# UCSD-Comp-Imaging/Nerf-Simple

Measured on AMD Instinct MI355X. Metric: ray-samples/sec at 800x800x128, higher is better.
Workload: dtype f16

## Files before the change

### nerf-simple_amd/csrc/mlp_bf16_16.hip

```cpp
#include "composite_device.h"
#include "launchers.h"

using namespace nerf_layout;

#ifdef NERF_HALF
typedef _Float16 elem_t;
#define NERF_MFMA __builtin_amdgcn_mfma_f32_16x16x32_f16
#define NERF_KERNEL nerf_mlp_f16_16_kernel
#define NERF_LAUNCH nerf_amd_launch_mlp_f16_16
#else
typedef __bf16 elem_t;
#define NERF_MFMA __builtin_amdgcn_mfma_f32_16x16x32_bf16
#define NERF_KERNEL nerf_mlp_bf16_16_kernel
#define NERF_LAUNCH nerf_amd_launch_mlp_bf16_16
#endif
#include "mlp16_chain.h"

namespace {

#ifdef NERF_HALF
constexpr bool FOLD = true;
#else
constexpr bool FOLD = false;
#endif
struct MlpPlan {
    static constexpr int LAYERS = NUM_LAYERS;
    static constexpr bool SAVE = !FOLD;
    static constexpr int tpc(int L) { return L == 0 ? 8 : 4; }
    static constexpr int mt(int L) { return FOLD ? fold_mt(L) : b16_mt(L); }
    static constexpr int layer_off_kib(int L) { return FOLD ? fold_layer_off_kib(L) : b16_layer_off_kib(L); }
    static constexpr int bias_off(int L) { return FOLD ? fold_bias_off(L) : b16_bias_off(L); }
};
static_assert(NUM_CHUNKS<MlpPlan> == (FOLD ? 34 : 38) && plan_fits<MlpPlan>(), "chunks per tile / weight buffer, parity");

constexpr int LDS_POSD = LDS_CHAIN_END;
constexpr int LDS_POSX = LDS_POSD + WAVES * NCB * 1024;
constexpr int LDS_TOTAL = LDS_POSX + WAVES * NCB * 2048;
constexpr int RING_PTS = 1024;
constexpr int LDS_RING_RAW = LDS_TOTAL;
constexpr int LDS_RING_T = LDS_RING_RAW + RING_PTS * 16;
constexpr int LDS_TOTAL_COMP = LDS_RING_T + RING_PTS * 4;
constexpr int COMP_MAX_N = RING_PTS - TILE_PTS;
static_assert(COMP_MAX_N == FUSED_RENDER_MAX_N, "api.hip routes by this limit");
static_assert(LDS_TOTAL_COMP <= 160 * 1024, "LDS budget");
static_assert((RING_PTS & (RING_PTS - 1)) == 0 && RING_PTS % TILE_PTS == 0, "ring indexing");

static_assert(ACT_TILE_PTS == TILE_PTS && MASK_TILE_PTS == TILE_PTS, "activation blocks and mask tiles are the kernel's tiles");

struct State {
    using Plan = MlpPlan;
    ex8 X[NCB][8], Y[NCB][8];
    f32x4 pend[NCB][2];
    float sigma[NCB], rgb[NCB][3];
    bool bad;
    unsigned posd_off[NCB];
    char* acts;
    long long P;
    long long tile;
    int loff[NCB];
    unsigned mb[NCB][2];
    float amax[4];
    long long mask_tile;
    long long p_end;
    unsigned ring_q0;
    WFrag* wf;
};

template <bool RAYS, int SAVE, bool COMP>
__device__ __forceinline__ void stage_inputs(const Ctx& c, const MlpArgs& a, long long tile_base, State& st) {
    const int col = c.lane & 15, g = c.lane >> 4;
    float u_mine = 0.f;
    bool dev_rng = false;
    long long b0 = 0;
    int r0 = 0;
    if constexpr (RAYS) {
        b0 = tile_base / a.N;
        r0 = (int)(tile_base - b0 * a.N);
    }
    const long long p_end = COMP ? st.p_end : a.P;
    const int last_local = (int)(p_end - 1 - tile_base);
    constexpr bool RAY_POSD = RAYS && !SAVE;
    if constexpr (RAY_POSD) {
        const int top = last_local < TILE_PTS - 1 ? last_local : TILE_PTS - 1;
        const int nrays = (int)(split_point(b0, r0, top, a.N).b - b0) + 1;
        for (int idx = threadIdx.x; idx < nrays * 32; idx += WAVES * 64) {
            const int ray = idx >> 5, slot = idx & 31, gg = slot >> 3, sl = slot & 7;
            const float* rp = a.rays + (b0 + ray) * 6 + 3;
            const float dx = rp[0], dy = rp[1], dz = rp[2];
            const float nrm = norm3(dx, dy, dz);
            float val = 0.f;
            if (sl < 6) {
                const int cd = sl >> 1;
                const float dc = __fdiv_rn(cd == 0 ? dx : cd == 1 ? dy : dz, nrm);
                val = enc_lane(to_revolutions(dc), 2 * gg + (sl & 1));
            } else if (sl == 6 && gg < 3) {
                val = __fdiv_rn(gg == 0 ? dx : gg == 1 ? dy : dz, nrm);
            }
            lds_store<elem_t>(LDS_POSD + ray * 64 + slot * 2, 0, (elem_t)val);
        }
    }
    if constexpr (RAYS && NCB == 2) {
        dev_rng = (a.flags & NERF_FLAG_DEVICE_RNG) && !(a.flags & NERF_FLAG_TS_GIVEN);
        if (dev_rng) {
            int lm = c.wave * 32 + (c.lane & 31);
            if (lm > last_local) lm = last_local;
            u_mine = device_rng_uniform(a, split_point(b0, r0, lm, a.N));
        }
    }
#pragma unroll
    for (int cb = 0; cb < NCB; ++cb) {
        long long p = tile_base + c.wave * (16 * NCB) + cb * 16 + col;
        const bool valid = p < p_end;
        st.loff[cb] = valid ? block_lane_offset(g, c.wave * (16 * NCB) + cb * 16 + col) : LOFF_INVALID;
        if constexpr (SAVE == 2) {
            if (cb == 0)
                st.loff[0] = tile_base + c.wave * 32 + 16 * (c.lane >> 5) + col < p_end ? f8_lane_offset(c.lane, c.wave) : LOFF_INVALID;
        }
        if (!valid) p = p_end - 1;
        PointIn pt;
        st.posd_off[cb] = c.b_posd + cb * 1024;
        if constexpr (RAYS) {
            const float u_cb = (NCB == 2) ? __shfl(u_mine, cb * 16 + col) : 0.f;
            int lp = c.wave * (16 * NCB) + cb * 16 + col;
            if (lp > last_local) lp = last_local;
            if (SAVE && a.pts) {
                pt = fetch_point_pts(a, p);
            } else {
                const RaySample rs = split_point(b0, r0, lp, a.N);
                if constexpr (RAY_POSD) st.posd_off[cb] = LDS_POSD + (unsigned)(rs.b - b0) * 64 + g * 16;
                pt = fetch_point_rays<!RAY_POSD>(a, p, rs, u_cb, dev_rng);
                if constexpr (COMP) {
                    if (valid && g == 0)
                        lds_store<float>(((st.ring_q0 + c.wave * (16 * NCB) + cb * 16 + col) & (RING_PTS - 1)) * 4, LDS_RING_T, pt.t);
                }
                if (valid && g == 0 && a.ts_out) a.ts_out[p] = pt.t;
            }
        } else {
            pt = fetch_point_pts(a, p);
        }
        {
            const float xyz[3] = {pt.x, pt.y, pt.z};
            float v[16];
#pragma unroll
            for (int cd = 0; cd < 3; ++cd) {
                const TwoF q = to_revolutions(xyz[cd]);
#pragma unroll
                for (int jj = 0; jj < 5; ++jj) v[cd * 5 + jj] = enc_lane(q, 5 * g + jj);
            }
            v[15] = g == 0 ? pt.x : g == 1 ? pt.y : g == 2 ? pt.z : 0.f;
#pragma unroll
            for (int e = 0; e < 2; ++e) {
                u32x4 r;
#pragma unroll
                for (int i = 0; i < 4; ++i) r[i] = pack2<false>(v[8 * e + 2 * i], v[8 * e + 2 * i + 1]);
                lds_store<u32x4>(c.b_posx, cb * 2048 + e * 1024, r);
            }
        }
        if constexpr (!RAY_POSD) {
            const float dd[3] = {pt.d1, pt.d2, pt.d3};
            float v[8];
#pragma unroll
            for (int cd = 0; cd < 3; ++cd) {
                const TwoF q = to_revolutions(dd[cd]);
#pragma unroll
                for (int jj = 0; jj < 2; ++jj) v[cd * 2 + jj] = enc_lane(q, 2 * g + jj);
            }
            v[6] = g == 0 ? pt.d1 : g == 1 ? pt.d2 : g == 2 ? pt.d3 : 0.f;
            v[7] = 0.f;
            u32x4 r;
#pragma unroll
            for (int i = 0; i < 4; ++i) r[i] = pack2<false>(v[2 * i], v[2 * i + 1]);
            lds_store<u32x4>(c.b_posd, cb * 1024, r);
        }
    }
}

template <bool RAYS, int SAVE, bool COMP>
__device__ __forceinline__ void run_tile(const Ctx& c, const MlpArgs& a, long long tile_base, State& st) {
    stage_inputs<RAYS, SAVE, COMP>(c, a, tile_base, st);
    run_layer<0, SAVE>(c, st, st.X, st.X);
    run_layer<1, SAVE>(c, st, st.X, st.Y);
    run_layer<2, SAVE>(c, st, st.Y, st.X);
    run_layer<3, SAVE>(c, st, st.X, st.Y);
    run_layer<4, SAVE>(c, st, st.Y, st.X);
    run_layer<5, SAVE>(c, st, st.X, st.Y);
    run_layer<6, SAVE>(c, st, st.Y, st.X);
    run_layer<7, SAVE>(c, st, st.X, st.Y);
    ex8 (&c_in)[NCB][8] = FOLD ? st.Y : st.X;
    ex8 (&c_out)[NCB][8] = FOLD ? st.X : st.Y;
    run_layer<8, SAVE>(c, st, st.Y, st.X);
    run_layer<9, SAVE>(c, st, c_in, c_out);
    run_layer<10, SAVE>(c, st, c_out, c_in);
    epilogue_piece<10, 0>(0, st.pend, st.X, st);
    for (int cb_ = 1; cb_ < NCB; ++cb_) epilogue_piece<10, 0>(4 * cb_, st.pend, st.X, st);
}

__device__ __forceinline__ bool finite4(float x, float y, float z, float w) {
    return __builtin_fabsf(x) + __builtin_fabsf(y) + __builtin_fabsf(z) + __builtin_fabsf(w) < __builtin_inff();
}

struct RingSamples {
    unsigned q0;
    __device__ __forceinline__ float t(int i) const {
        return lds_load<float>(((q0 + (unsigned)i) & (RING_PTS - 1)) * 4, LDS_RING_T);
    }
    __device__ __forceinline__ f32x4 c(int i) const {
        return lds_load<f32x4>(((q0 + (unsigned)i) & (RING_PTS - 1)) * 16, LDS_RING_RAW);
    }
};

template <bool RAYS, int SAVE, bool COMP>
__device__ __forceinline__ void kernel_body(const MlpArgs& a, long long ntiles) {
    static_assert(!COMP || (RAYS && !SAVE), "the fused render is the rays-mode inference kernel");
    using P = MlpPlan;
    Ctx c;
    c.wave = __builtin_amdgcn_readfirstlane(threadIdx.x >> 6);
    c.lane = threadIdx.x & 63;
    const char* img = reinterpret_cast<const char*>(a.packed);
    c.wrsrc = __builtin_amdgcn_make_buffer_rsrc(const_cast<char*>(img), 0, (int)B16_IMAGE_BYTES, 0x00020000);
    c.wave_goff = c.wave * 1024;
    c.lane16 = c.lane * 16;
#pragma unroll
    for (int p = 0; p < 2; ++p) {
        c.b_wread[p] = LDS_W0 + p * LDS_WBUF + c.lane * 16;
        c.s_wdst[p] = LDS_W0 + p * LDS_WBUF + c.wave * 1024;
    }
    c.b_bias = (c.lane >> 4) * 16;
    c.b_posx = LDS_POSX + c.wave * (NCB * 2048) + c.lane * 16;
    c.b_posd = LDS_POSD + c.wave * (NCB * 1024) + c.lane * 16;

    {
        const float* bsrc = reinterpret_cast<const float*>(img + (long long)B16_WEIGHT_KIB * 1024);
        for (int i = threadIdx.x; i < B16_BIAS_FLOATS; i += WAVES * 64)
            lds_store<float>(i * 4, LDS_BIAS, bsrc[i]);
        Stage<P, NUM_CHUNKS<P> - 1>::issue(c);
    }
    asm volatile("s_waitcnt vmcnt(0)" ::: "memory");
    __syncthreads();
    WFrag wf;
    {
        constexpr int F0 = chunk_tiles<P>(0) * (layer_desc(0).chain_k / 32 + layer_desc(0).extra_slots / 32);
#pragma unroll
        for (int f = 0; f < 4 && f < F0; ++f) wf.a[f] = lds_load<ex8>(c.b_wread[0], f * 1024);
        wf.bias0 = lds_load<f32x4>(c.b_bias, LDS_BIAS + P::bias_off(0) * 4);
    }

    if constexpr (!COMP) {
        for (long long tile = blockIdx.x; tile < ntiles; tile += gridDim.x) {
            const long long tile_base = tile * TILE_PTS;
            asm volatile("" : "+s"(c.wave_goff));
            State st;
            st.wf = &wf;
            st.acts = reinterpret_cast<char*>(a.acts);
            st.P = a.P;
            st.mask_tile = SAVE == 2 ? f8_mask_offset_bytes(0, tile, 0, a.P) : mask_offset_bytes(0, tile, 0, a.P);
            st.tile = tile;
            st.bad = false;
            run_tile<RAYS, SAVE, false>(c, a, tile_base, st);
            bool bad = st.bad;
            if (c.lane < 16) {
#pragma unroll
                for (int cb = 0; cb < NCB; ++cb) {
                    const long long p = tile_base + c.wave * (16 * NCB) + cb * 16 + c.lane;
                    if (p < a.P) {
                        const f32x4 o = {st.rgb[cb][0], st.rgb[cb][1], st.rgb[cb][2], st.sigma[cb]};
                        *reinterpret_cast<f32x4*>(a.raw + p * 4) = o;
                        bad |= !finite4(o[0], o[1], o[2], o[3]);
                    }
                }
            }
            flag_nonfinite(c, bad);
        }
    } else {
        const long long B = a.P / a.N;
        const long long r_lo = (long long)blockIdx.x * B / gridDim.x, r_hi = ((long long)blockIdx.x + 1) * B / gridDim.x;
        const long long range_base = r_lo * a.N;
        const int n_pts = (int)((r_hi - r_lo) * a.N);
        const nerf_composite::RayOut out{a.rgb, a.disp, a.alpha, a.acc, a.w, a.pixels};
        int next_ray = 0, n_complete = 0;
        for (int q_tile = 0; q_tile < n_pts; q_tile += TILE_PTS) {
            const long long tile_base = range_base + q_tile;
            asm volatile("" : "+s"(c.wave_goff));
            State st;
            st.wf = &wf;
            st.acts = nullptr;
            st.P = a.P;
            st.mask_tile = 0;
            st.tile = 0;
            st.p_end = range_base + n_pts;
            st.ring_q0 = (unsigned)q_tile & (RING_PTS - 1);
            st.bad = false;
            run_tile<true, false, true>(c, a, tile_base, st);
            bool bad = st.bad;
            if (c.lane < 16) {
#pragma unroll
                for (int cb = 0; cb < NCB; ++cb) {
                    const int local = c.wave * (16 * NCB) + cb * 16 + c.lane;
                    if (q_tile + local < n_pts) {
                        const f32x4 o = {st.rgb[cb][0], st.rgb[cb][1], st.rgb[cb][2], st.sigma[cb]};
                        lds_store<f32x4>(((st.ring_q0 + local) & (RING_PTS - 1)) * 16, LDS_RING_RAW, o);
                        bad |= !finite4(o[0], o[1], o[2], o[3]);
                    }
                }
            }
            flag_nonfinite(c, bad);
            asm volatile("s_waitcnt lgkmcnt(0)" ::: "memory");
            __builtin_amdgcn_s_barrier();
            asm volatile("" ::: "memory");
            const int done_q = q_tile + TILE_PTS < n_pts ? q_tile + TILE_PTS : n_pts;
            while ((n_complete + 1) * a.N <= done_q) ++n_complete;
            if (n_complete - next_ray >= WAVES || done_q + TILE_PTS - next_ray * a.N > RING_PTS || done_q == n_pts) {
                for (int ray = next_ray + c.wave; ray < n_complete; ray += WAVES) {
                    const long long gray = r_lo + ray;
                    const float* d = a.rays + gray * 6 + 3;
                    const float dnorm = nerf_composite::unit_dir_norm(d[0], d[1], d[2], true);
                    const RingSamples src{(unsigned)(ray * a.N) & (RING_PTS - 1)};
                    nerf_composite::composite_ray(src, a.N, c.lane, dnorm, gray, out);
                }
                next_ray = n_complete;
                asm volatile("s_waitcnt lgkmcnt(0)" ::: "memory");
                __builtin_amdgcn_s_barrier();
                asm volatile("" ::: "memory");
            }
        }
    }
}

template <bool RAYS, bool SAVE, bool COMP>
__global__ __launch_bounds__(WAVES * 64, WAVES / 4) void NERF_KERNEL(MlpArgs a, long long ntiles) {
    extern __shared__ __attribute__((aligned(16))) char smem[];
    (void)smem;
    kernel_body<RAYS, SAVE ? 1 : 0, COMP>(a, ntiles);
}
#ifndef NERF_HALF
__global__ __launch_bounds__(WAVES * 64, WAVES / 4) void nerf_mlp_train_e4m3_kernel(MlpArgs a, long long ntiles) {
    extern __shared__ __attribute__((aligned(16))) char smem[];
    (void)smem;
    kernel_body<true, 2, false>(a, ntiles);
}
#endif

}

extern "C" int NERF_LAUNCH(const MlpArgs* args, int rays_mode, hipStream_t stream) {
    (void)hipGetLastError();
    MlpArgs a = *args;
    if (a.P <= 0) return 0;
    const long long ntiles = (a.P + TILE_PTS - 1) / TILE_PTS;
    const int cus = device_cus();
    const long long grid = ntiles < cus ? ntiles : cus;
    hipError_t e = hipSuccess;
    const bool comp = a.rgb || a.disp || a.acc || a.alpha || a.w || a.pixels;
    if (comp) {
        if (!rays_mode || a.acts || a.N > COMP_MAX_N || a.P / grid + a.N >= (1ll << 31)) return -2;
        auto kern = NERF_KERNEL<true, false, true>;
        e = allow_dynamic_lds(reinterpret_cast<const void*>(kern), LDS_TOTAL_COMP);
        if (e != hipSuccess) return (int)e;
        hipLaunchKernelGGL(kern, dim3((unsigned)grid), dim3(WAVES * 64), LDS_TOTAL_COMP, stream, a, ntiles);
        return (int)hipGetLastError();
    }
#ifdef NERF_HALF
    if (a.acts) return -2;
    auto kern = rays_mode ? NERF_KERNEL<true, false, false> : NERF_KERNEL<false, false, false>;
#else
    if (a.acts && !rays_mode) return -2;
    if ((a.flags & NERF_FLAG_STORE_E4M3) && !a.acts) return -2;
    auto kern = a.acts ? ((a.flags & NERF_FLAG_STORE_E4M3) ? nerf_mlp_train_e4m3_kernel : NERF_KERNEL<true, true, false>)
                       : (rays_mode ? NERF_KERNEL<true, false, false> : NERF_KERNEL<false, false, false>);
#endif
    e = allow_dynamic_lds(reinterpret_cast<const void*>(kern), LDS_TOTAL);
    if (e != hipSuccess) return (int)e;
    hipLaunchKernelGGL(kern, dim3((unsigned)grid), dim3(WAVES * 64), LDS_TOTAL, stream, a, ntiles);
    return (int)hipGetLastError();
}
```

### nerf-simple_amd/csrc/nerf_device.h

```cpp
#pragma once
#include <hip/hip_runtime.h>
#include <stdint.h>
#include <atomic>
#include "nerf_layout.h"

typedef __bf16 bf16x8 __attribute__((ext_vector_type(8)));
typedef __bf16 bf16x2 __attribute__((ext_vector_type(2)));
typedef short s16x2 __attribute__((ext_vector_type(2)));
typedef unsigned short u16x2 __attribute__((ext_vector_type(2)));
typedef float f32x2 __attribute__((ext_vector_type(2)));
typedef float f32x4 __attribute__((ext_vector_type(4)));
typedef float f32x16 __attribute__((ext_vector_type(16)));
typedef unsigned u32x4 __attribute__((ext_vector_type(4)));

#define NERF_FLAG_TS_GIVEN 1u
#define NERF_FLAG_DEVICE_RNG 2u
#define NERF_FLAG_SEED_IN_MEMORY 4u
#define NERF_FLAG_STORE_E4M3 8u

struct MlpArgs {
    const float* pts;
    const float* rays;
    const float* u;
    const float* tbins;
    const void* packed;
    float* raw;
    float* ts_out;
    void* acts;
    long long P;
    long long ray_id0;
    unsigned long long seed;
    int N;
    unsigned flags;
    float* rgb;
    float* disp;
    float* alpha;
    float* acc;
    float* w;
    float* pixels;
};

struct DensityArgs {
    const float* pts;
    long long stride;
    const void* packed;
    float* sigma;
    long long P;
    long long ny, nz;
    float lo[3], step[3];
};

constexpr int NERF_MAX_DEVICES = 64;
inline int device_cus() {
    static int cache[NERF_MAX_DEVICES] = {};
    int dev = 0;
    if (hipGetDevice(&dev) != hipSuccess || dev < 0 || dev >= NERF_MAX_DEVICES) return 256;
    if (cache[dev] == 0) {
        int cus = 256;
        if (hipDeviceGetAttribute(&cus, hipDeviceAttributeMultiprocessorCount, dev) != hipSuccess || cus <= 0) cus = 256;
        cache[dev] = cus;
    }
    return cache[dev];
}
inline hipError_t allow_dynamic_lds(const void* kernel, int bytes) {
    struct Slot { const void* kernel; int dev; };
    static Slot slots[128];
    static std::atomic<int> used{0};
    int dev = 0;
    if (hipGetDevice(&dev) != hipSuccess) dev = -1;
    const int n = used.load(std::memory_order_acquire);
    for (int i = 0; i < n && i < 128; ++i)
        if (slots[i].kernel == kernel && slots[i].dev == dev) return hipSuccess;
    const hipError_t e = hipFuncSetAttribute(kernel, hipFuncAttributeMaxDynamicSharedMemorySize, bytes);
    if (e == hipSuccess && dev >= 0) {
        const int i = used.load(std::memory_order_relaxed);
        if (i < 128) {
            slots[i] = Slot{kernel, dev};
            used.store(i + 1, std::memory_order_release);
        }
    }
    return e;
}

constexpr int LOFF_INVALID = 0x40000000;
__host__ __device__ constexpr int swapped_chunk(int g) { return (g & 1) * 2 + (g >> 1); }
__host__ __device__ constexpr int block_lane_offset(int g, int local) { return swapped_chunk(g) * 4096 + local * 16; }

template <int AUX = 0>
__device__ __forceinline__ void store_granule(__amdgpu_buffer_rsrc_t rs, int voffset, int soffset, u32x4 w) {
    const auto s0 = __builtin_amdgcn_permlane16_swap(w[0], w[2], false, false);
    const auto s1 = __builtin_amdgcn_permlane16_swap(w[1], w[3], false, false);
    const unsigned o0 = s0[0], o1 = s1[0], o2 = s0[1], o3 = s1[1];
    __builtin_amdgcn_raw_buffer_store_b128(u32x4{o0, o1, o2, o3}, rs, voffset, soffset, AUX);
    asm volatile("s_nop 1" ::"v"(o0), "v"(o1), "v"(o2), "v"(o3) : "memory");
}

template <bool ABS>
__device__ __forceinline__ float f8_absmax(float running, float v0, float v1) {
    float r;
    if constexpr (ABS) asm("v_max3_f32 %0, %1, |%2|, |%3|" : "=v"(r) : "v"(running), "v"(v0), "v"(v1));
    else asm("v_max3_f32 %0, %1, %2, %3" : "=v"(r) : "v"(running), "v"(v0), "v"(v1));
    return r;
}
__device__ __forceinline__ int f8_wave_max_exponent(float m) {
    int r;
    asm volatile("s_nop 1\n\t"
                 "v_max_f32_dpp %1, %1, %1 quad_perm:[1,0,3,2] row_mask:0xf bank_mask:0xf\n\ts_nop 1\n\t"
                 "v_max_f32_dpp %1, %1, %1 quad_perm:[2,3,0,1] row_mask:0xf bank_mask:0xf\n\ts_nop 1\n\t"
                 "v_max_f32_dpp %1, %1, %1 row_half_mirror row_mask:0xf bank_mask:0xf\n\ts_nop 1\n\t"
                 "v_max_f32_dpp %1, %1, %1 row_mirror row_mask:0xf bank_mask:0xf\n\ts_nop 1\n\t"
                 "v_max_f32_dpp %1, %1, %1 row_bcast:15 row_mask:0xa bank_mask:0xf\n\ts_nop 1\n\t"
                 "v_max_f32_dpp %1, %1, %1 row_bcast:31 row_mask:0xc bank_mask:0xf\n\ts_nop 1\n\t"
                 "v_readlane_b32 %0, %1, 63"
                 : "=s"(r), "+v"(m));
    return (r >> 23) & 0xff;
}
__device__ __forceinline__ unsigned f8_cvt4(unsigned lo, unsigned hi, float scale) {
    unsigned r;
    asm("v_cvt_scalef32_pk_fp8_bf16 %0, %1, %3\n\tv_cvt_scalef32_pk_fp8_bf16 %0, %2, %3 op_sel:[0,0,1]"
        : "=&v"(r) : "v"(lo), "v"(hi), "s"(scale));
    return r;
}
__host__ __device__ constexpr int f8_lane_offset(int lane, int wave) {
    return ((lane >> 4) & 1) * 4096 + (wave * 32 + 16 * (lane >> 5) + (lane & 15)) * 16;
}
template <int AUX = 0>
__device__ __forceinline__ void store_fragment_f8(__amdgpu_buffer_rsrc_t rs_data, int voff, int soff_data, u32x4 w0, u32x4 w1,
                                                  float scale) {
    const unsigned a0 = f8_cvt4(w0[0], w0[1], scale), b0 = f8_cvt4(w0[2], w0[3], scale);
    unsigned a1 = f8_cvt4(w1[0], w1[1], scale), b1 = f8_cvt4(w1[2], w1[3], scale);
    asm volatile("s_nop 1" : "+v"(a1), "+v"(b1));
    const auto x0 = __builtin_amdgcn_permlane32_swap(a0, a1, false, false);
    const auto x1 = __builtin_amdgcn_permlane32_swap(b0, b1, false, false);
    const auto y0 = __builtin_amdgcn_permlane16_swap(x0[0], x1[0], false, false);
    const auto y1 = __builtin_amdgcn_permlane16_swap(x0[1], x1[1], false, false);
    const unsigned o0 = y0[0], o1 = y0[1], o2 = y1[0], o3 = y1[1];
#if defined(F8_TIMING) && F8_TIMING == 2
    asm volatile("" ::"v"(o0), "v"(o1), "v"(o2), "v"(o3));
#else
    __builtin_amdgcn_raw_buffer_store_b128(u32x4{o0, o1, o2, o3}, rs_data, voff, soff_data,
#if defined(F8_TIMING) && F8_TIMING == 3
                                           0);
#else
                                           AUX);
#endif
    asm volatile("s_nop 1" ::"v"(o0), "v"(o1), "v"(o2), "v"(o3) : "memory");
#endif
}
constexpr int F8_GROUP = 4;
template <int AUX = 0>
__device__ __forceinline__ void store_group_f8(__amdgpu_buffer_rsrc_t rs_data, int voff, int soff_data,
                                               __amdgpu_buffer_rsrc_t rs_scale, int lane, int scale_byte,
                                               const u32x4 (&w0)[F8_GROUP], const u32x4 (&w1)[F8_GROUP], float amax) {
#if defined(F8_TIMING) && F8_TIMING == 1
    const int e = (__builtin_bit_cast(int, amax) >> 23) & 0xff;
#else
    const int e = f8_wave_max_exponent(amax);
#endif
    const int sb = e > 8 ? e - 7 : 1;
    const float scale = __builtin_bit_cast(float, sb << 23);
#pragma unroll
    for (int k = 0; k < F8_GROUP; ++k) store_fragment_f8<AUX>(rs_data, voff, soff_data + k * 8192, w0[k], w1[k], scale);
#if !(defined(F8_TIMING) && F8_TIMING == 2)
    __builtin_amdgcn_raw_buffer_store_b32((unsigned)sb * 0x01010101u, rs_scale, lane == 0 ? scale_byte : LOFF_INVALID, 0, 0);
#endif
}

template <int N>
__device__ __forceinline__ void chunk_barrier() {
    asm volatile("s_waitcnt vmcnt(%0)" ::"n"(N) : "memory");
    __builtin_amdgcn_s_barrier();
    asm volatile("" ::: "memory");
}

__device__ __forceinline__ void wave_lds_fence() {
    __builtin_amdgcn_s_waitcnt(0xc07f);
    __builtin_amdgcn_wave_barrier();
}

typedef __attribute__((address_space(3))) char lds_char;
typedef __attribute__((address_space(3))) void lds_void;
template <class T>
__device__ __forceinline__ T lds_load(unsigned base, int imm) {
    return *reinterpret_cast<const __attribute__((address_space(3))) T*>(reinterpret_cast<lds_char*>(0) + base + imm);
}
template <class T>
__device__ __forceinline__ void lds_store(unsigned base, int imm, const T& v) {
    *reinterpret_cast<__attribute__((address_space(3))) T*>(reinterpret_cast<lds_char*>(0) + base + imm) = v;
}

template <class C, int NEXT, int KIB, int OFF_KIB, int WAVES>
struct ChunkDma {
    static constexpr int PIECES = (KIB + WAVES - 1) / WAVES;
    static constexpr int SRC_OFF = OFF_KIB * 1024;
    static __device__ __forceinline__ void issue_piece(const C& c, int p) {
        __builtin_amdgcn_raw_ptr_buffer_load_lds(
            c.wrsrc, reinterpret_cast<lds_void*>(reinterpret_cast<lds_char*>(0) + c.s_wdst[NEXT & 1] + p * (WAVES * 1024)), 16,
            c.lane16, c.wave_goff + (SRC_OFF + p * WAVES * 1024), 0, 0);
    }
    static __device__ __forceinline__ void issue(const C& c) {
#pragma unroll
        for (int p = 0; p < PIECES; ++p) issue_piece(c, p);
    }
};

__device__ __forceinline__ unsigned philox_word(unsigned long long seed, unsigned long long ctr) {
    unsigned c0 = (unsigned)ctr, c1 = (unsigned)(ctr >> 32), c2 = 0x6e657266u, c3 = 0x616d6421u;
    unsigned k0 = (unsigned)seed, k1 = (unsigned)(seed >> 32);
#pragma unroll
    for (int r = 0; r < 10; ++r) {
        const unsigned long long p0 = 0xD2511F53ull * c0, p1 = 0xCD9E8D57ull * c2;
        const unsigned n0 = (unsigned)(p1 >> 32) ^ c1 ^ k0, n2 = (unsigned)(p0 >> 32) ^ c3 ^ k1;
        c1 = (unsigned)p1; c3 = (unsigned)p0; c0 = n0; c2 = n2;
        k0 += 0x9E3779B9u; k1 += 0xBB67AE85u;
    }
    return c0;
}
__device__ __forceinline__ float philox_uniform(unsigned long long seed, unsigned long long ctr) {
    return (float)(philox_word(seed, ctr) >> 8) * (1.0f / 16777216.0f);
}

__device__ __forceinline__ float mul_rn(float a, float b) {
#pragma clang fp contract(off)
    return a * b;
}
__device__ __forceinline__ float add_rn(float a, float b) {
#pragma clang fp contract(off)
    return a + b;
}
__device__ __forceinline__ float sub_rn(float a, float b) {
#pragma clang fp contract(off)
    return a - b;
}
__device__ __forceinline__ float sqrt_rn(float a) { return sqrtf(a); }

__device__ __forceinline__ float norm3(float x, float y, float z) {
    return sqrt_rn(__fmaf_rn(z, z, __fmaf_rn(y, y, mul_rn(x, x))));
}

struct PointIn {
    float x, y, z, d1, d2, d3, t;
};

struct RaySample { long long b; int i; };
__device__ __forceinline__ RaySample split_point(long long b0, int r0, int local, int N) {
    const unsigned tt = (unsigned)(r0 + local);
    unsigned q = (unsigned)((float)tt * __frcp_rn((float)N));
    if ((long long)q * N > (long long)tt) --q;
    if ((long long)(q + 1) * N <= (long long)tt) ++q;
    return RaySample{b0 + q, (int)(tt - q * (unsigned)N)};
}
__device__ __forceinline__ RaySample split_point(long long p, int N) {
    const long long b = p / N;
    return RaySample{b, (int)(p - b * N)};
}

__device__ __forceinline__ unsigned long long effective_seed(const MlpArgs& a) {
    if (!(a.flags & NERF_FLAG_SEED_IN_MEMORY)) return a.seed;
    const unsigned long long v = *reinterpret_cast<const unsigned long long*>(a.u);
    const unsigned lo = __builtin_amdgcn_readfirstlane((unsigned)v), hi = __builtin_amdgcn_readfirstlane((unsigned)(v >> 32));
    return a.seed + (((unsigned long long)hi << 32) | lo);
}

__device__ __forceinline__ float device_rng_uniform(const MlpArgs& a, RaySample rs) {
    unsigned long long seed = effective_seed(a);
    asm volatile("" : "+s"(seed));
    return philox_uniform(seed, (unsigned long long)((a.ray_id0 + rs.b) * a.N + rs.i));
}

template <bool DIR = true>
__device__ __forceinline__ PointIn fetch_point_rays(const MlpArgs& a, long long p, RaySample rs, float u_pre = 0.f,
                                                    bool have_u = false) {
    PointIn r;
    const long long b = rs.b;
    const int i = rs.i;
    const float* ray = a.rays + b * 6;
    const float ox = ray[0], oy = ray[1], oz = ray[2];
    const float dx = ray[3], dy = ray[4], dz = ray[5];
    float t;
    if (a.flags & NERF_FLAG_TS_GIVEN) {
        t = __builtin_nontemporal_load(a.u + p);
    } else {
        float u;
        if (a.flags & NERF_FLAG_DEVICE_RNG)
            u = have_u ? u_pre : philox_uniform(effective_seed(a), (unsigned long long)((a.ray_id0 + b) * a.N + i));
        else
            u = __builtin_nontemporal_load(a.u + p);
        const float bin_diff = sub_rn(a.tbins[1], a.tbins[0]);
        t = add_rn(mul_rn(bin_diff, u), a.tbins[i]);
    }
    r.t = t;
    r.x = add_rn(ox, mul_rn(dx, t));
    r.y = add_rn(oy, mul_rn(dy, t));
    r.z = add_rn(oz, mul_rn(dz, t));
    if constexpr (DIR) {
        const float nrm = norm3(dx, dy, dz);
        r.d1 = __fdiv_rn(dx, nrm);
        r.d2 = __fdiv_rn(dy, nrm);
        r.d3 = __fdiv_rn(dz, nrm);
    } else {
        r.d1 = r.d2 = r.d3 = 0.f;
    }
    return r;
}

__device__ __forceinline__ PointIn fetch_point_rays(const MlpArgs& a, long long p) {
    return fetch_point_rays(a, p, split_point(p, a.N));
}

__device__ __forceinline__ PointIn fetch_point_pts(const MlpArgs& a, long long p) {
    PointIn r;
    const float* v = a.pts + p * 6;
    r.x = v[0]; r.y = v[1]; r.z = v[2];
    r.d1 = v[3]; r.d2 = v[4]; r.d3 = v[5];
    r.t = 0.f;
    return r;
}

struct TwoF { float hi, lo; };
__device__ __forceinline__ TwoF to_revolutions(float x) {
    const float C_HI = 0.15915494f;
    const float C_LO = 6.4206382e-09f;
    x = __builtin_amdgcn_fmed3f(x, -0x1p100f, 0x1p100f);
    TwoF q;
    q.hi = mul_rn(x, C_HI);
    const float err = __fmaf_rn(x, C_HI, -q.hi);
    q.lo = __fmaf_rn(x, C_LO, err);
    return q;
}
__device__ __forceinline__ float enc_lane(TwoF q, int idx) {
    const float sc = __builtin_amdgcn_ldexpf(1.0f, idx >> 1);
    const float fr = __builtin_amdgcn_fractf(q.hi * sc) + q.lo * sc + ((idx & 1) ? 0.25f : 0.f);
    return __builtin_amdgcn_sinf(fr);
}
__device__ __forceinline__ void sincos_rev_fast(TwoF q, float scale, float& s, float& c) {
    const float f = __builtin_amdgcn_fractf(q.hi * scale) + q.lo * scale;
    s = __builtin_amdgcn_sinf(f);
    c = __builtin_amdgcn_cosf(f);
}
```

Measured before the change: 1.355 billion.

## Specialize render-path input staging with hoisted launch constants and early-issued loads

Result: no change. 1.354 billion (-0.0%).

```diff
diff --git a/nerf-simple_amd/csrc/mlp_bf16_16.hip b/nerf-simple_amd/csrc/mlp_bf16_16.hip
--- a/nerf-simple_amd/csrc/mlp_bf16_16.hip
+++ b/nerf-simple_amd/csrc/mlp_bf16_16.hip
@@ -63,11 +63,147 @@
     long long mask_tile;
     long long p_end;
     unsigned ring_q0;
+    const struct RenderLaunch* rl;
+    int q_tile, b_rel, r0;
     WFrag* wf;
 };
 
+__device__ __forceinline__ void store_posx(const Ctx& c, int cb, int g, const PointIn& pt) {
+    const float xyz[3] = {pt.x, pt.y, pt.z};
+    float v[16];
+#pragma unroll
+    for (int cd = 0; cd < 3; ++cd) {
+        const TwoF q = to_revolutions(xyz[cd]);
+#pragma unroll
+        for (int jj = 0; jj < 5; ++jj) v[cd * 5 + jj] = enc_lane(q, 5 * g + jj);
+    }
+    v[15] = g == 0 ? pt.x : g == 1 ? pt.y : g == 2 ? pt.z : 0.f;
+#pragma unroll
+    for (int e = 0; e < 2; ++e) {
+        u32x4 r;
+#pragma unroll
+        for (int i = 0; i < 4; ++i) r[i] = pack2<false>(v[8 * e + 2 * i], v[8 * e + 2 * i + 1]);
+        lds_store<u32x4>(c.b_posx, cb * 2048 + e * 1024, r);
+    }
+}
+
+__device__ __forceinline__ void store_ray_posd(int ray, int slot, float dx, float dy, float dz) {
+    const int gg = slot >> 3, sl = slot & 7;
+    const float nrm = norm3(dx, dy, dz);
+    float val = 0.f;
+    if (sl < 6) {
+        const int cd = sl >> 1;
+        const float dc = __fdiv_rn(cd == 0 ? dx : cd == 1 ? dy : dz, nrm);
+        val = enc_lane(to_revolutions(dc), 2 * gg + (sl & 1));
+    } else if (sl == 6 && gg < 3) {
+        val = __fdiv_rn(gg == 0 ? dx : gg == 1 ? dy : dz, nrm);
+    }
+    lds_store<elem_t>(LDS_POSD + ray * 64 + slot * 2, 0, (elem_t)val);
+}
+
+struct RenderLaunch {
+    const float* rays_lo;
+    const float* u_lo;
+    unsigned long long ctr_base;
+    unsigned long long seed;
+    float bin_diff;
+    int jitter;
+    int n_pts;
+    int step_b, step_r;
+};
+__device__ __forceinline__ float uniform_f32(float x) {
+    return __builtin_bit_cast(float, __builtin_amdgcn_readfirstlane(__builtin_bit_cast(unsigned, x)));
+}
+__device__ __forceinline__ RenderLaunch render_launch(const MlpArgs& a, long long r_lo, long long range_base, int n_pts) {
+    RenderLaunch rl;
+    rl.jitter = (a.flags & NERF_FLAG_TS_GIVEN) ? JITTER_TS_GIVEN : (a.flags & NERF_FLAG_DEVICE_RNG) ? JITTER_DEVICE_RNG : JITTER_U_GIVEN;
+    rl.rays_lo = a.rays + r_lo * 6;
+    rl.u_lo = rl.jitter != JITTER_DEVICE_RNG ? a.u + range_base : nullptr;
+    rl.ctr_base = (unsigned long long)(a.ray_id0 * a.N + range_base);
+    rl.seed = rl.jitter == JITTER_DEVICE_RNG ? effective_seed(a) : 0ull;
+    rl.bin_diff = rl.jitter != JITTER_TS_GIVEN ? uniform_f32(sub_rn(a.tbins[1], a.tbins[0])) : 0.f;
+    rl.n_pts = n_pts;
+    rl.step_b = TILE_PTS / a.N;
+    rl.step_r = TILE_PTS - rl.step_b * a.N;
+    return rl;
+}
+__device__ __forceinline__ void next_tile(const RenderLaunch& rl, int N, int& b_rel, int& r0) {
+    b_rel += rl.step_b;
+    r0 += rl.step_r;
+    if (r0 >= N) { r0 -= N; ++b_rel; }
+}
+
+template <int J>
+__device__ __forceinline__ void stage_inputs_render(const Ctx& c, const MlpArgs& a, State& st) {
+    static_assert(NCB == 2, "a lane's Philox draw serves the wave's 32 points");
+    const RenderLaunch& rl = *st.rl;
+    int tid = threadIdx.x;
+    asm volatile("" : "+v"(tid));
+    const int lane = tid & 63, col = lane & 15, g = lane >> 4;
+    const int N = a.N;
+    const int last_local = rl.n_pts - 1 - st.q_tile;
+    const int top = last_local < TILE_PTS - 1 ? last_local : TILE_PTS - 1;
+    const int nrays = (int)split_point(0, st.r0, top, N).b + 1;
+    const float* tile_rays = rl.rays_lo + (long long)st.b_rel * 6;
+    int lp[NCB];
+    RaySample rs[NCB];
+#pragma unroll
+    for (int cb = 0; cb < NCB; ++cb) {
+        lp[cb] = c.wave * (16 * NCB) + cb * 16 + col;
+        if (lp[cb] > last_local) lp[cb] = last_local;
+        rs[cb] = split_point(0, st.r0, lp[cb], N);
+    }
+    int idx = tid;
+    float dir[3];
+    {
+        const int ray = (idx >> 5) < nrays ? (idx >> 5) : nrays - 1;
+        const float* rp = at_bytes(tile_rays, (unsigned)ray * 24u + 12u);
+        dir[0] = rp[0]; dir[1] = rp[1]; dir[2] = rp[2];
+    }
+    PointLoads pl[NCB];
+#pragma unroll
+    for (int cb = 0; cb < NCB; ++cb)
+        pl[cb] = issue_point_rays<J>(at_bytes(tile_rays, (unsigned)rs[cb].b * 24u), at_bytes(a.tbins, (unsigned)rs[cb].i * 4u),
+                                     at_bytes(rl.u_lo, (unsigned)(st.q_tile + lp[cb]) * 4u));
+    float u_mine = 0.f;
+    if constexpr (J == JITTER_DEVICE_RNG) {
+        int lm = c.wave * 32 + (lane & 31);
+        if (lm > last_local) lm = last_local;
+        __builtin_amdgcn_sched_barrier(0);
+        u_mine = device_rng_uniform(rl.seed, rl.ctr_base + (unsigned)(st.q_tile + lm));
+    }
+    asm volatile("" : "+v"(dir[0]), "+v"(dir[1]), "+v"(dir[2]), "+v"(u_mine));
+    if (idx < nrays * 32) store_ray_posd(idx >> 5, idx & 31, dir[0], dir[1], dir[2]);
+    for (idx += WAVES * 64; idx < nrays * 32; idx += WAVES * 64) {
+        const float* rp = at_bytes(tile_rays, (unsigned)(idx >> 5) * 24u + 12u);
+        store_ray_posd(idx >> 5, idx & 31, rp[0], rp[1], rp[2]);
+    }
+#pragma unroll
+    for (int cb = 0; cb < NCB; ++cb) {
+        const int local = c.wave * (16 * NCB) + cb * 16 + col;
+        const bool valid = local <= last_local;
+        st.loff[cb] = valid ? block_lane_offset(g, local) : LOFF_INVALID;
+        st.posd_off[cb] = LDS_POSD + (unsigned)rs[cb].b * 64 + g * 16;
+        const float u_cb = J == JITTER_DEVICE_RNG ? __shfl(u_mine, cb * 16 + col) : 0.f;
+        const PointIn pt = finish_point_rays<J>(pl[cb], rl.bin_diff, u_cb);
+        if (valid && g == 0) {
+            lds_store<float>(((st.ring_q0 + local) & (RING_PTS - 1)) * 4, LDS_RING_T, pt.t);
+            if (a.ts_out) a.ts_out[st.p_end - rl.n_pts + st.q_tile + local] = pt.t;
+        }
+        store_posx(c, cb, g, pt);
+    }
+}
+
 template <bool RAYS, int SAVE, bool COMP>
 __device__ __forceinline__ void stage_inputs(const Ctx& c, const MlpArgs& a, long long tile_base, State& st) {
+    if constexpr (COMP) {
+        switch (st.rl->jitter) {
+            case JITTER_DEVICE_RNG: stage_inputs_render<JITTER_DEVICE_RNG>(c, a, st); break;
+            case JITTER_U_GIVEN: stage_inputs_render<JITTER_U_GIVEN>(c, a, st); break;
+            default: stage_inputs_render<JITTER_TS_GIVEN>(c, a, st); break;
+        }
+        return;
+    }
     const int col = c.lane & 15, g = c.lane >> 4;
     float u_mine = 0.f;
     bool dev_rng = false;
@@ -77,7 +213,7 @@
         b0 = tile_base / a.N;
         r0 = (int)(tile_base - b0 * a.N);
     }
-    const long long p_end = COMP ? st.p_end : a.P;
+    const long long p_end = a.P;
     const int last_local = (int)(p_end - 1 - tile_base);
     constexpr bool RAY_POSD = RAYS && !SAVE;
     if constexpr (RAY_POSD) {
@@ -129,10 +265,6 @@
                 const RaySample rs = split_point(b0, r0, lp, a.N);
                 if constexpr (RAY_POSD) st.posd_off[cb] = LDS_POSD + (unsigned)(rs.b - b0) * 64 + g * 16;
                 pt = fetch_point_rays<!RAY_POSD>(a, p, rs, u_cb, dev_rng);
-                if constexpr (COMP) {
-                    if (valid && g == 0)
-                        lds_store<float>(((st.ring_q0 + c.wave * (16 * NCB) + cb * 16 + col) & (RING_PTS - 1)) * 4, LDS_RING_T, pt.t);
-                }
                 if (valid && g == 0 && a.ts_out) a.ts_out[p] = pt.t;
             }
         } else {
@@ -277,7 +409,9 @@
         const long long range_base = r_lo * a.N;
         const int n_pts = (int)((r_hi - r_lo) * a.N);
         const nerf_composite::RayOut out{a.rgb, a.disp, a.alpha, a.acc, a.w, a.pixels};
+        const RenderLaunch rl = render_launch(a, r_lo, range_base, n_pts);
         int next_ray = 0, n_complete = 0;
+        int b_rel = 0, r0 = 0;
         for (int q_tile = 0; q_tile < n_pts; q_tile += TILE_PTS) {
             const long long tile_base = range_base + q_tile;
             asm volatile("" : "+s"(c.wave_goff));
@@ -289,6 +423,10 @@
             st.tile = 0;
             st.p_end = range_base + n_pts;
             st.ring_q0 = (unsigned)q_tile & (RING_PTS - 1);
+            st.rl = &rl;
+            st.q_tile = q_tile;
+            st.b_rel = b_rel;
+            st.r0 = r0;
             st.bad = false;
             run_tile<true, false, true>(c, a, tile_base, st);
             bool bad = st.bad;
@@ -322,6 +460,7 @@
                 __builtin_amdgcn_s_barrier();
                 asm volatile("" ::: "memory");
             }
+            next_tile(rl, a.N, b_rel, r0);
         }
     }
 }
diff --git a/nerf-simple_amd/csrc/nerf_device.h b/nerf-simple_amd/csrc/nerf_device.h
--- a/nerf-simple_amd/csrc/nerf_device.h
+++ b/nerf-simple_amd/csrc/nerf_device.h
@@ -308,6 +308,47 @@
     return fetch_point_rays(a, p, split_point(p, a.N));
 }
 
+enum { JITTER_DEVICE_RNG = 0, JITTER_U_GIVEN = 1, JITTER_TS_GIVEN = 2 };
+template <class T>
+__device__ __forceinline__ const T* at_bytes(const T* base, unsigned off) {
+    return reinterpret_cast<const T*>(reinterpret_cast<const char*>(base) + off);
+}
+struct PointLoads {
+    float o[3], d[3];
+    float tbin;
+    float uj;
+};
+template <int J>
+__device__ __forceinline__ PointLoads issue_point_rays(const float* ray, const float* tbin_i, const float* uj) {
+    PointLoads l;
+#pragma unroll
+    for (int k = 0; k < 3; ++k) { l.o[k] = ray[k]; l.d[k] = ray[3 + k]; }
+    l.tbin = J != JITTER_TS_GIVEN ? *tbin_i : 0.f;
+    l.uj = J != JITTER_DEVICE_RNG ? __builtin_nontemporal_load(uj) : 0.f;
+    return l;
+}
+template <int J>
+__device__ __forceinline__ PointIn finish_point_rays(const PointLoads& l, float bin_diff, float u_dev) {
+    PointIn r;
+    float t;
+    if constexpr (J == JITTER_TS_GIVEN) {
+        t = l.uj;
+    } else {
+        const float u = J == JITTER_DEVICE_RNG ? u_dev : l.uj;
+        t = add_rn(mul_rn(bin_diff, u), l.tbin);
+    }
+    r.t = t;
+    r.x = add_rn(l.o[0], mul_rn(l.d[0], t));
+    r.y = add_rn(l.o[1], mul_rn(l.d[1], t));
+    r.z = add_rn(l.o[2], mul_rn(l.d[2], t));
+    r.d1 = r.d2 = r.d3 = 0.f;
+    return r;
+}
+__device__ __forceinline__ float device_rng_uniform(unsigned long long seed, unsigned long long ctr) {
+    asm volatile("" : "+s"(seed));
+    return philox_uniform(seed, ctr);
+}
+
 __device__ __forceinline__ PointIn fetch_point_pts(const MlpArgs& a, long long p) {
     PointIn r;
     const float* v = a.pts + p * 6;
```
